# DaviGuanabara/dronechase

Measured on AMD Instinct MI355X. Metric: env-steps/sec (whole job), random-action rollout, higher is better.
Workload: dtype f32

## Files before the change

### dronechase_amd/csrc/te_engage_slots.hpp

```cpp
#pragma once
#include "te_engage.hpp"

namespace te {

constexpr int kSlotWaves = 16;
constexpr int kSlotPursuers = 4;

struct SlotRows {
  int D, P;
  TE_DEV int accS() const { return 0; }
  TE_DEV int accZone() const { return 1; }
  TE_DEV int accOrg() const { return 2; }
  TE_DEV int accOwn() const { return 3; }
  TE_DEV int pos(int k, int s) const { return 4 + k * D + s; }
  TE_DEV int cellr(int s) const { return 4 + 3 * D + 2 * s; }
  TE_DEV int npos(int k, int s) const { return 4 + (5 + k) * D + s; }
  TE_DEV int prec(int q) const { return 4 + 8 * D + q; }
  TE_DEV int prec2(int q) const { return 4 + 8 * D + 2 * q; }
};
__host__ __device__ inline int slot_lds_rows(int D, int P) { return 4 + 8 * D + 2 * P; }
enum : uint32_t { SLOT_HIT = 1u << 8, SLOT_EXPLODE = 1u << 9, SLOT_SUICIDE = 1u << 10 };

#define TE_SLOT_BARRIER() asm volatile("s_waitcnt lgkmcnt(0)\n\ts_barrier" ::: "memory")
#if defined(TE_DEBUG_STAMPS)
#define TE_WSTAMP(idx, wait)                                                                                              \
  do {                                                                                                                    \
    if (wait) asm volatile("s_waitcnt vmcnt(0) lgkmcnt(0)" ::: "memory");                                                 \
    if (p.dbg && s < 2 && lane == 0) p.dbg[64 + blockIdx.x * 16 + s * 8 + (idx)] = __builtin_amdgcn_s_memrealtime();     \
  } while (0)
#else
#define TE_WSTAMP(idx, wait) do {} while (0)
#endif

template <int DM>
__global__ __launch_bounds__(DM * 64) __attribute__((amdgpu_waves_per_eu(6, 10))) void engage_slots_kernel(Params p, const float* __restrict__ actions, StepOut o) {
  TE_EXACT
  extern __shared__ uint32_t sm[];
  const te_config& c = p.cfg;
  const int D = p.D, P = c.n_pursuers;
  const SlotRows R{D, P};
  const int lane = threadIdx.x & 63;
  const int s = __builtin_amdgcn_readfirstlane((int)(threadIdx.x >> 6));
  const int env = blockIdx.x * 64 + lane;
  const bool valid = env < p.N;
  const GView g{p.dstate, p.estate, D, p.Npad, env, P};
  const EnvIO io(p, env);
  const uint32_t pur_bits = (1u << P) - 1u, all_bits = (1u << D) - 1u, inv_bits = all_bits & ~pur_bits;
  const bool scripted = all_scripted(c);
  const bool is_p = s < P;
  auto L = [&](int row) -> uint32_t& { return sm[row * 64 + lane]; };
  auto Lf = [&](int row) { return __uint_as_float(sm[row * 64 + lane]); };
  auto Lor = [&](int row, uint32_t v) { __hip_atomic_fetch_or(&sm[row * 64 + lane], v, __ATOMIC_RELAXED, __HIP_MEMORY_SCOPE_WORKGROUP); };
  TE_WSTAMP(0, 0);

  const uint32_t* __restrict__ lm32 = reinterpret_cast<const uint32_t*>(p.live_mask);
  const uint32_t live = (uint32_t)__builtin_amdgcn_readfirstlane(lm32[2 * blockIdx.x]) & all_bits;
  const bool mine_live = is_p || ((live >> s) & 1u);
  auto next_round_of = [&](int r) { return r + (r < c.n_rounds ? 1 : c.n_rounds); };
  auto may_be_spawned = [&](int slot, int r) { const int i = slot - P; return i < invaders_in_round(c, next_round_of(r)) || i < invaders_in_round(c, 1); };
  if (!mine_live) {
    const int r = (int)io.le(TE_E_ROUND);
    if (__ballot(valid && may_be_spawned(s, r)) == 0ull) return;
  }
  float mx = io.ldf(TE_D_OBS_POS, s), my = io.ldf(TE_D_OBS_POS + 1, s), mz = io.ldf(TE_D_OBS_POS + 2, s);
  const uint32_t marmed_w = io.ld(TE_D_ARMED, s);
  const V3 apos{io.ldf(TE_D_OBS_POS, 0), io.ldf(TE_D_OBS_POS + 1, 0), io.ldf(TE_D_OBS_POS + 2, 0)};
  float ag[9];
#pragma unroll
  for (int k = 0; k < 3; ++k) ag[k] = io.ldf(TE_D_OBS_EULER + k, 0);
#pragma unroll
  for (int k = 3; k < 9; ++k) ag[k] = 0.0f;
  const uint32_t w_step = io.le(TE_E_STEP), w_max_step = io.le(TE_E_MAX_STEP), w_round = io.le(TE_E_ROUND), w_episode = io.le(TE_E_EPISODE);
  uint32_t w_last_dist = 0u, w_ak = 0u, w_lk = 0u, w_dd = 0u;
  float4 act = make_float4(0.0f, 0.0f, 0.0f, 0.0f);
  if (s == 0) {
#pragma unroll
    for (int k = 3; k < 9; ++k) ag[k] = io.ldf(TE_D_OBS_EULER + k, 0);
    w_last_dist = io.le(TE_E_LAST_DIST); w_ak = io.le(TE_E_AGENT_KILLS); w_lk = io.le(TE_E_ALLIES_KILLS); w_dd = io.le(TE_E_DEADS);
    if (valid) act = reinterpret_cast<const float4*>(actions)[env];
  }
  uint32_t w_mun = 0u, w_lf = 0u; float fx = 0.0f, fy = 0.0f, fz = 0.0f;
  if (is_p) {
    w_mun = io.ld(TE_D_MUNITION, s); w_lf = io.ld(TE_D_LAST_FIRED, s);
    fx = io.ldf(TE_D_FORMATION, s); fy = io.ldf(TE_D_FORMATION + 1, s); fz = io.ldf(TE_D_FORMATION + 2, s);
  }
  uint32_t zero = 0u;
  asm volatile("" : "+s"(zero));
  if (s == 0) { L(R.accS()) = 0u; L(R.accZone()) = 0u; L(R.accOrg()) = 0u; L(R.accOwn()) = 0u; }
  TE_SLOT_BARRIER();
  int step = (int)w_step + 1;
  int max_step = (int)w_max_step, round = (int)w_round;
  uint32_t episode = w_episode;
  int mun = (int)w_mun, lf = (int)w_lf;
  const float last_dist = __uint_as_float(w_last_dist);
  int agent_kills = (int)w_ak, allies_kills = (int)w_lk, deads = (int)w_dd;
  if (!mine_live) { mx = my = mz = 0.0f; }
  TE_WSTAMP(1, 1);

  const uint32_t a_me = (mine_live && marmed_w != zero && valid) ? 1u : 0u;
  {
    const float n = fnorm(V3{mx, my, mz});
    Lor(R.accS(), a_me << s); Lor(R.accZone(), (a_me & (n > c.dome_radius ? 1u : 0u)) << s); Lor(R.accOrg(), (a_me & (n < c.origin_range ? 1u : 0u)) << s);
    L(R.pos(0, s)) = __float_as_uint(mx); L(R.pos(1, s)) = __float_as_uint(my); L(R.pos(2, s)) = __float_as_uint(mz);
  }
  int cj = 0; float rh = 1.0f;
  if (s >= 1) {
    const M3 Rm = x_inverse_attitude(ag[0], ag[1], ag[2]);
    lidar_cell_fast(c, x_mul(Rm, sub(V3{mx, my, mz}, apos)), cj, rh);
    *reinterpret_cast<uint2*>(&sm[R.cellr(s) * 64 + 2 * lane]) = make_uint2((uint32_t)cj, __float_as_uint(rh));
  }
  TE_WSTAMP(2, 0);
  TE_SLOT_BARRIER();
  TE_WSTAMP(3, 0);
  const uint32_t S = L(R.accS()), zone = L(R.accZone()), org = L(R.accOrg());
  if (is_p) {
    int tgt = -1; float dmin = 0.0f;
    for (uint32_t m = live & inv_bits; m; m &= m - 1u) {
      const int j = __ffs((int)m) - 1;
      const float d = fdist(V3{mx, my, mz}, V3{Lf(R.pos(0, j)), Lf(R.pos(1, j)), Lf(R.pos(2, j))});
      const bool take = a_me != 0u && ((S >> j) & 1u) != 0u && (tgt < 0 || d < dmin);
      tgt = take ? j : tgt;
      dmin = take ? d : dmin;
    }
    uint32_t rec = (uint32_t)(tgt + 1);
    if (a_me && tgt >= 0 && dmin < c.shoot_range && gun_available(c, mun, lf, step) && mun > 0) {
      mun -= 1; lf = step;
      io.st(TE_D_MUNITION, s, (uint32_t)mun); io.st(TE_D_LAST_FIRED, s, (uint32_t)step);
      const U4 r = env_rng(c, env, RNG_HIT, (uint32_t)s, 0, episode, (uint32_t)step);
      if (u01(r.x) < c.hit_prob) {
        rec |= SLOT_HIT;
        if (c.evaluation) g.si(TE_D_KILLS, s, g.gi(TE_D_KILLS, s) + 1);
      }
    }
    if (a_me && tgt >= 0 && dmin < c.explosion_range) rec |= SLOT_EXPLODE | (mun == 0 ? SLOT_SUICIDE : 0u);
    L(R.prec(s)) = rec;
  }
  TE_SLOT_BARRIER();

  uint32_t killed = 0u;
  int agent_shots = 0, ally_shots = 0, exploded = 0, pursuer_suicided = 0, agent_suicided = 0;
  for (int q = 0; q < P; ++q) {
    const uint32_t r = L(R.prec(q));
    const int t = (int)(r & 0xFFu) - 1;
    if (r & SLOT_HIT) { killed |= 1u << t; if (q == 0) agent_shots += 1; else ally_shots += 1; }
    if (r & SLOT_EXPLODE) {
      killed |= (1u << q) | (1u << t);
      if ((r & SLOT_SUICIDE) && q == 0) agent_suicided += 1;
      else if (r & SLOT_SUICIDE) pursuer_suicided += 1;
      else exploded += 1;
    }
  }
  if ((!c.evaluation || (c.evaluation & TE_EVAL_ORIGIN_RULE)) && valid) killed |= org & inv_bits;
  const uint32_t A = S & ~killed;
  if ((killed >> s) & 1u) io.disarm(s);
  if (agent_shots + ally_shots > 0) max_step += c.step_increment;
  const int armed_invaders = __popc(A & inv_bits), armed_pursuers = __popc(A & pur_bits);
  const bool all_rounds_over = armed_invaders == 0 && round >= c.n_rounds;
  bool term;
  if (c.evaluation) term = (c.max_step > 0 && step > max_step) || all_rounds_over || zone != 0u || armed_pursuers == 0;
  else term = step > max_step || all_rounds_over || zone != 0u || armed_pursuers == 0 || (c.agent_death_terminates && !(A & 1u)) || apos.z < -5.99f;
  const bool to_terminal = valid && term && c.auto_reset;
  bool own = false;
  if (s >= 1) {
    own = ((A >> s) & 1u) != 0u && rh < 1.0f;
    for (uint32_t m = live & ~1u & ~(1u << s); m; m &= m - 1u) {
      const int k = __ffs((int)m) - 1;
      const uint2 cr = *reinterpret_cast<const uint2*>(&sm[R.cellr(k) * 64 + 2 * lane]);
      const float rk = __uint_as_float(cr.y);
      const bool beaten = ((A >> k) & 1u) != 0u && cr.x == (uint32_t)cj && (rk < rh || (rk == rh && k < s));
      own = own && !beaten;
    }
    if (own && valid) Lor(R.accOwn(), 1u << s);
  }
  const float flag_me = (float)(s < P ? TE_TYPE_LOYALWINGMAN : TE_TYPE_LOITERINGMUNITION) / 5.0f;
  const bool time_plane = c.lidar_channels != 2;
  auto patch = [&](float* dst) {
    dst += (size_t)env * lidar_words(c);
    dst[cj] = rh; dst[TE_LIDAR_CELLS + cj] = flag_me;
    if (time_plane) dst[2 * TE_LIDAR_CELLS + cj] = 0.1f;
  };
  if (valid && own && !to_terminal && o.obs.lidar) patch(o.obs.lidar);
  const unsigned long long term_b = __ballot(to_terminal);
  if (o.term.lidar && term_b && is_p) {
    for (unsigned long long tb = term_b; tb; tb &= tb - 1) {
      const int l = __ffsll((long long)tb) - 1;
      float* tile = o.term.lidar + (size_t)(blockIdx.x * 64 + l) * lidar_words(c);
      for (int e = s * 64 + lane; e < lidar_words(c); e += 64 * P) tile[e] = 1.0f;
    }
  }

  auto pos_of = [&](int t) { return V3{__uint_as_float(sm[R.pos(0, t) * 64 + lane]), __uint_as_float(sm[R.pos(1, t) * 64 + lane]), __uint_as_float(sm[R.pos(2, t) * 64 + lane])}; };
  if (s == 0) {
    if (valid) {
      io.stef(TE_E_LAST_ACTION + 0, act.x); io.stef(TE_E_LAST_ACTION + 1, act.y); io.stef(TE_E_LAST_ACTION + 2, act.z); io.stef(TE_E_LAST_ACTION + 3, act.w);
      io.ste(TE_E_STEP, (uint32_t)step);
      io.ste(TE_E_SNAP_MASK, S); io.ste(TE_E_SNAP_MASK_HI, 0u);
    }
    agent_kills += agent_shots; allies_kills += ally_shots; deads += exploded;
    if (to_terminal) {
      if (o.term.inertial) inertial_row_regs(c, o.term.inertial + (size_t)env * TE_OBS_INERTIAL_WORDS, mx, my, mz, ag, mun, lf, step);
      if (o.term.last_action) reinterpret_cast<float4*>(o.term.last_action)[env] = act;
    }
    float reward = 0.0f, cur_dist = last_dist;
    if (!c.evaluation) {
      float gs[3];
      gun_state(c, mun, lf, step, max_munition_of(c, 0), gs);
      const float dist_origin = fnorm(apos);
      int ally = -1;
      if ((S & 1u) && __popc(S & pur_bits) > 1) {
        float bd = 0.0f;
        for (int a = 1; a < P; ++a) {
          if ((S >> a) & 1u) {
            const float d = fdist(pos_of(a), apos);
            if (ally < 0 || d < bd) { ally = a; bd = d; }
          }
        }
      }
      const int chooser = ally < 0 ? 0 : ally;
      const int target = ((S >> chooser) & 1u) ? (int)(sm[R.prec(chooser) * 64 + lane] & 0xFFu) - 1 : -1;
      const V3 tp = target >= 0 ? pos_of(target) : V3{0.0f, 0.0f, 0.0f};
      cur_dist = fdist(apos, tp);
      const bool ready = gs[2] == 1.0f || gs[0] == 0.0f;
      float bonus = 0.0f, penalty = 0.0f;
      if (0.01f < last_dist - cur_dist && ready) bonus += c.approach_bonus_gain * fnorm(V3{ag[3], ag[4], ag[5]});
      const float score = ready ? -cur_dist : cur_dist * (2.0f * gs[1] - 1.0f);
      if (agent_shots > 0 || agent_suicided > 0) bonus += (float)(agent_shots + agent_suicided) * 1000.0f;
      if (ally_shots > 0 || pursuer_suicided > 0) bonus += 0.5f * (float)(ally_shots + pursuer_suicided) * 1000.0f;
      else if (exploded > 0) penalty += 1000.0f * (float)exploded;
      if (apos.z < -5.0f) penalty += (-5.0f - apos.z) * 1000.0f;
      if (zone & pur_bits) penalty += 1000.0f;
      if (dist_origin > c.born_radius - 2.0f) penalty += dist_origin - c.born_radius - 2.0f;
      reward = score + bonus - penalty;
    }
    if (valid) {
      if (!c.evaluation) io.stef(TE_E_LAST_DIST, cur_dist);
      io.ste(TE_E_AGENT_KILLS, (uint32_t)agent_kills); io.ste(TE_E_ALLIES_KILLS, (uint32_t)allies_kills); io.ste(TE_E_DEADS, (uint32_t)deads);
      if (agent_shots + ally_shots > 0) io.ste(TE_E_MAX_STEP, (uint32_t)max_step);
      o.reward[env] = reward;
      o.done[env] = term ? 1 : 0;
      reinterpret_cast<int4*>(o.info)[env] = make_int4(agent_kills, allies_kills, deads, round);
      io.ste(TE_E_INFO_WAVE, (uint32_t)round);
    }
  }

  uint32_t task = 0u;
  uint32_t snap_mask = S;
  auto mask_after_spawn = [&](int rnd, bool reset) {
    const uint32_t m = reset ? pur_bits : (A & pur_bits);
    const int n = invaders_in_round(c, rnd);
    return (uint32_t)(m | ((((1u << n) - 1u) << P) & all_bits));
  };
  if (valid && !term && armed_invaders == 0 && armed_pursuers > 0) {
    round = round + (round < c.n_rounds ? 1 : c.n_rounds);
    snap_mask = mask_after_spawn(round, false);
    if (s == 0) { io.ste(TE_E_ROUND, (uint32_t)round); io.ste(TE_E_SNAP_MASK, snap_mask); io.ste(TE_E_SNAP_MASK_HI, 0u); }
    task = (uint32_t)round;
  }
  if (to_terminal) {
    episode += 1u; step = 0; max_step = c.max_step; round = 1;
    snap_mask = mask_after_spawn(1, true);
    if (s == 0) {
      io.ste(TE_E_EPISODE, episode); io.ste(TE_E_STEP, 0u); io.ste(TE_E_MAX_STEP, (uint32_t)c.max_step); io.ste(TE_E_ROUND, 1u); io.ste(TE_E_INFO_WAVE, 1u);
      io.ste(TE_E_AGENT_KILLS, 0u); io.ste(TE_E_ALLIES_KILLS, 0u); io.ste(TE_E_DEADS, 0u);
      if (c.reward_model != TE_REWARD_L5_C1) io.stef(TE_E_LAST_DIST, c.dome_radius);
#pragma unroll
      for (int k = 0; k < 4; ++k) io.ste(TE_E_LAST_ACTION + k, 0u);
      io.ste(TE_E_SNAP_MASK, snap_mask); io.ste(TE_E_SNAP_MASK_HI, 0u);
    }
    act = make_float4(0.0f, 0.0f, 0.0f, 0.0f);
#pragma unroll
    for (int k = 0; k < 9; ++k) ag[k] = 0.0f;
    task = 1u | (1u << 8);
  }
  if (task != 0u) {
    const bool reset = (task >> 8) != 0u;
    V3 w{0.0f, 0.0f, 0.0f};
    const bool placed = io.spawn_uniform(c, env, s, (int)(task & 0xFFu), episode, reset, ((A >> s) & 1u) != 0u, w);
    if (placed) { mx = w.x; my = w.y; mz = w.z; }
    if (reset && is_p) { mun = max_munition_of(c, s); lf = -c.cooldown_steps; fx = mx; fy = my; fz = mz; }
  }
  if (s == 0 && __ballot(task != 0u) != 0ull) {
    for (uint32_t m = inv_bits & ~live; m; m &= m - 1u) {
      const int k2 = __ffs((int)m) - 1;
      if (__ballot(valid && may_be_spawned(k2, (int)w_round)) != 0ull) continue;
      if (task != 0u) io.st(TE_D_NAV_STATE, k2, (uint32_t)TE_NAV_WAIT);
    }
  }
  const uint32_t armed_post = task != 0u ? snap_mask : A;
  L(R.npos(0, s)) = __float_as_uint(mx); L(R.npos(1, s)) = __float_as_uint(my); L(R.npos(2, s)) = __float_as_uint(mz);
  if (o.term.lidar && term_b) asm volatile("s_waitcnt vmcnt(0)" ::: "memory");
  TE_WSTAMP(4, 0);
  TE_SLOT_BARRIER();
  TE_WSTAMP(5, 0);

  if (s >= 1 && to_terminal && own && o.term.lidar) patch(o.term.lidar);
  if (o.persist && o.obs.lidar && valid) {
    const uint32_t owners = L(R.accOwn());
    uint16_t* pv = o.prev + env;
    if (s == 0) pv[0] = (uint16_t)(to_terminal ? 0 : __popc(owners));
    else if (own && !to_terminal) pv[(size_t)(__popc(owners & ((1u << s) - 1u)) + 1) * p.Npad] = (uint16_t)cj;
  }
  if (s == 0) {
    if (o.obs.inertial && valid) inertial_row_regs(c, o.obs.inertial + (size_t)env * TE_OBS_INERTIAL_WORDS, mx, my, mz, ag, mun, lf, step);
    if (valid && o.obs.last_action) reinterpret_cast<float4*>(o.obs.last_action)[env] = act;
  }
  if (is_p && valid) {
    int first_skipped = -1;
    if (!scripted && !(armed_post & 1u)) first_skipped = (armed_post & pur_bits & ~1u) ? __ffs((int)(armed_post & pur_bits & ~1u)) - 1 : -1;
    io.stf(TE_X_REF + 0, s, mx); io.stf(TE_X_REF + 1, s, my); io.stf(TE_X_REF + 2, s, mz);
    if ((s > 0 || scripted) && ((armed_post >> s) & 1u) && s != first_skipped) {
      float out[3] = {0.0f, 0.0f, 0.0f};
      const bool ext = driven_externally(c, s);
      if (!ext && c.ally_policy == TE_ALLY_BT) {
        const V3 me{mx, my, mz};
        if (gun_available(c, mun, lf, step)) {
          int t = -1; float bd = 0.0f; V3 tp{0.0f, 0.0f, 0.0f};
          if ((snap_mask >> s) & 1u) {
            for (int j = P; j < D; ++j) {
              if (__ballot((snap_mask >> j) & 1u) == 0ull) continue;
              if ((snap_mask >> j) & 1u) {
                const V3 pj{Lf(R.npos(0, j)), Lf(R.npos(1, j)), Lf(R.npos(2, j))};
                const float d = fdist(me, pj);
                if (t < 0 || d < bd) { t = j; bd = d; tp = pj; }
              }
            }
          }
          x_cmd_toward(me, tp, c.ally_speed, out);
        } else x_cmd_toward(me, V3{fx, fy, fz}, c.ally_speed, out);
      } else if (ext || c.ally_policy != TE_ALLY_FROZEN) {
        out[0] = g.gf(TE_D_SETPOINT + 0, s); out[1] = g.gf(TE_D_SETPOINT + 1, s); out[2] = g.gf(TE_D_SETPOINT + 3, s);
      }
      io.stf(TE_X_CMD + 0, s, out[0]); io.stf(TE_X_CMD + 1, s, out[1]); io.stf(TE_X_CMD + 2, s, out[2]);
    }
  }
  const int writer = 0;
  if (s >= 1 || s == writer) {
    uint64_t dense = 0u, livem = 0u; int n = 0;
    uint16_t* items = p.mixed_items + (size_t)blockIdx.x * kMixedCap;
    const int k_last = s == writer ? D - 1 : s;
    for (int k = 0; k <= k_last; ++k) {
      const bool a = valid && ((armed_post >> k) & 1u) != 0u;
      const unsigned long long b = __ballot(a);
      const int cnt = __popcll(b);
      if (cnt == 0) continue;
      livem |= (uint64_t)1 << k;
      if (k == 0 || cnt >= p.dense_min || n + cnt > kMixedCap) { dense |= (uint64_t)1 << k; continue; }
      if (k == s && a) items[n + (int)__builtin_amdgcn_mbcnt_hi((uint32_t)(b >> 32), __builtin_amdgcn_mbcnt_lo((uint32_t)b, 0u))] = (uint16_t)(lane | (k << 8));
      n += cnt;
    }
    if (s == writer && lane == 0) { p.slot_mask[blockIdx.x] = dense; p.mixed_count[blockIdx.x] = (uint32_t)n; p.live_mask[blockIdx.x] = livem; }
  }
  TE_WSTAMP(6, 0);
  TE_WSTAMP(7, 1);
}

struct MultiSlotRows {
  int D, P, H;
  TE_DEV int accS(int h = 0) const { return h; }
  TE_DEV int accZone(int h = 0) const { return H + h; }
  TE_DEV int accOrg(int h = 0) const { return 2 * H + h; }
  TE_DEV int pos(int k, int s) const { return 3 * H + k * D + s; }
  TE_DEV int npos(int k, int s) const { return 3 * H + (3 + k) * D + s; }
  TE_DEV int prec(int q) const { return 3 * H + 6 * D + q; }
  TE_DEV int accOwn() const { return 3 * H + 6 * D + P; }
  TE_DEV int cellr(int s) const { return 3 * H + 1 + 6 * D + P + 2 * s; }
};
__host__ __device__ inline int multi_slot_lds_rows(int D, int P, bool lidar) { return 3 * (D > 32 ? 2 : 1) + 6 * D + P + (lidar ? 1 + 2 * D : 0); }

template <int SPW, bool LIDAR, bool WIDE = false>
__global__ __launch_bounds__(1024) __attribute__((amdgpu_waves_per_eu(SPW == 1 ? 4 : 6))) void engage_slots_multi_kernel(Params p, const float* __restrict__ actions, StepOut o) {
  TE_EXACT
  extern __shared__ uint32_t sm[];
  const te_config& c = p.cfg;
  const int D = p.D, P = c.n_pursuers;
  const int W = (int)(blockDim.x >> 6);
  using M = typename std::conditional<WIDE, uint64_t, uint32_t>::type;
  constexpr M one = 1;
  constexpr int kSh = WIDE ? 63 : 31;
  static_assert(!(WIDE && LIDAR), "the own sphere's owner row is 32 bits");
  const MultiSlotRows R{D, P, WIDE ? 2 : 1};
  auto popcM = [](M m) { return WIDE ? __popcll((unsigned long long)m) : __popc((uint32_t)m); };
  auto ffsM = [](M m) { return WIDE ? __ffsll((long long)m) - 1 : __ffs((int)(uint32_t)m) - 1; };
  const int lane = threadIdx.x & 63;
  const int s = __builtin_amdgcn_readfirstlane((int)(threadIdx.x >> 6));
  const int env = blockIdx.x * 64 + lane;
  const bool valid = env < p.N;
  const GView g{p.dstate, p.estate, D, p.Npad, env, P};
  const EnvIO io(p, env);
  const M pur_bits = (one << P) - one, all_bits = D >= (int)(8 * sizeof(M)) ? ~(M)0 : (one << D) - one, inv_bits = all_bits & ~pur_bits;
  const bool scripted = all_scripted(c);
  const bool is_p = s < P;
  int sl[SPW]; bool has[SPW];
#pragma unroll
  for (int u = 0; u < SPW; ++u) { sl[u] = s + u * W; has[u] = sl[u] < D; }
  auto L = [&](int row) -> uint32_t& { return sm[row * 64 + lane]; };
  auto Lf = [&](int row) { return __uint_as_float(sm[row * 64 + lane]); };
  auto Lor = [&](int row, uint32_t v) { __hip_atomic_fetch_or(&sm[row * 64 + lane], v, __ATOMIC_RELAXED, __HIP_MEMORY_SCOPE_WORKGROUP); };
  TE_WSTAMP(0, 0);

  const uint32_t* __restrict__ lm32 = reinterpret_cast<const uint32_t*>(p.live_mask);
  const M live = (WIDE ? (M)((uint64_t)(uint32_t)__builtin_amdgcn_readfirstlane(lm32[2 * blockIdx.x]) | ((uint64_t)(uint32_t)__builtin_amdgcn_readfirstlane(lm32[2 * blockIdx.x + 1]) << 32))
                       : (M)(uint32_t)__builtin_amdgcn_readfirstlane(lm32[2 * blockIdx.x])) & all_bits;
  auto next_round_of = [&](int r) { return r + (r < c.n_rounds ? 1 : c.n_rounds); };
// ... 639 lines not shown
```

### dronechase_amd/csrc/te_env.hip

```cpp
#include <hip/hip_runtime.h>
#include <hip/hip_ext.h>

#include <algorithm>
#include <cmath>
#include <cstdio>
#include <cstdlib>
#include <cstring>
#include <new>
#include <string>
#include <tuple>
#include <type_traits>
#include <vector>

#include "te_logic.hpp"
#include "te_stacked.hpp"
#include "te_stackview.hpp"
#include "te_engage.hpp"
#include "te_engage_slots.hpp"
#include "te_policy.hpp"
#include "te_wingman.hpp"
#include "te_policy_grad.hpp"
#include "te_policy_opt.hpp"
#include "te_rollout.hpp"
#include "te_monitor.hpp"
// ... 666 lines not shown
  if (cfg->task == TE_TASK_STAGE01 && !(cfg->n_pursuers == 2 && cfg->n_invaders == 1)) return "te_create: stage01 is 2 pursuers + 1 invader";
  if (cfg->lidar_radius <= 0.0f || cfg->dome_radius <= 0.0f || cfg->max_speed <= 0.0f) return "te_create: radii / max_speed must be positive";
  if (cfg->control_every_substep != 0 && cfg->control_every_substep != 1) return "te_create: control_every_substep is 0 or 1";
  if (cfg->lidar_channels != 3 && cfg->lidar_channels != 2) return "te_create: lidar_channels is 3 (distance, flag, time) or 2 (distance, flag)";
  if (cfg->lidar_channels == 2 && cfg->stacked_obs) return "te_create: the stacked observation (level5) always has 3 channels";
  if (cfg->io_location != TE_IO_DEVICE && cfg->io_location != TE_IO_HOST) return "te_create: io_location is TE_IO_DEVICE or TE_IO_HOST";
  if (cfg->io_location == TE_IO_HOST && (cfg->stacked_obs || cfg->ally_policy == TE_ALLY_EXTERNAL || ((uint32_t)cfg->evaluation >> 8) != 0u))
    return "te_create: TE_IO_HOST serves te_reset / te_observe / te_step / te_random_actions / te_get_state / te_set_state; the stacked observation and caller-driven wingmen take device pointers";
  if (cfg->drone_contact != 0 && cfg->drone_contact != 1) return "te_create: drone_contact is 0 or 1";
  if (cfg->drone_contact && !(cfg->contact_radius > 0.0f)) return "te_create: contact_radius must be positive";
  const size_t npad = ((size_t)cfg->n_envs + 63) / 64 * 64;
  if ((size_t)(TE_DRONE_WORDS + TE_X_WORDS) * D * npad >= (1ull << 30)) return "te_create: n_envs * drones too large for one te_env (state planes are indexed with 32 bits); shard it";
  return nullptr;
}

static const char* plan_kernels(const te_config& c, KernelPlan* out, size_t multi_lds_max = 160 * 1024) {
  KernelPlan& k = *out = KernelPlan{};
  const int P = c.n_pursuers, D = P + c.n_invaders, fam = family_of(c.task);
  const long long chunks = (c.n_envs + 63) / 64;
  const bool l4 = fam == FAM_LEVEL4, contact = c.drone_contact != 0;
  const char* engage = getenv("TE_ENGAGE");
  const bool eng_lds = engage && !strcmp(engage, "lds"), eng_regs = engage && !strcmp(engage, "regs");
  const bool regs_l4 = l4 && !eng_lds && P <= 7 && D <= 37;
  const bool regs_s2 = fam == FAM_STAGE02 && !eng_lds && P <= 2 && D <= 10;
  const bool regs_s1 = fam == FAM_STAGE01 && !eng_lds;
  if (D > kMaxD && !(regs_l4 && c.stacked_obs))
    return "te_create: more than 32 drones per env are served for the stacked-observation tasks only (te_step_stacked / te_step_students: stacked_obs, P <= 7, P + I <= 37)";
  if ((c.agent_scripted || c.reward_model != TE_REWARD_EXP03 || !c.agent_death_terminates || c.initial_invaders != 1 || c.invaders_per_round != 1) && !regs_l4)
    return "te_create: agent_scripted / reward_model / agent_death_terminates / the round rule are built into engage_kernel: the level4 task family with P <= 7 and P + I <= 37";
  if (contact && !(regs_l4 && P <= 6 && D <= 18))
    return "te_create: cfg.drone_contact is built into engage_kernel: the level4 task family with P <= 6 and P + I <= 18";
#ifdef TE_DEBUG_STAMPS
  if (contact) return "te_create: cfg.drone_contact is not served by the stamp build (TE_DEBUG_STAMPS leaves out the drone-contact engage kernels)";
#endif
  const bool slots = regs_l4 && !eng_regs && !c.stacked_obs && D <= kSlotWaves && P <= kSlotPursuers && c.reward_model == TE_REWARD_EXP03 && !contact;
  int spw = 0;
  const size_t multi_lds = (size_t)multi_slot_lds_rows(D, P, !c.stacked_obs) * 256;
  if (regs_l4 && !eng_regs && (D <= 32 || (c.stacked_obs && D <= 3 * kSlotWaves)) && !contact && (c.stacked_obs || D > kSlotWaves || slots)) {
    int s = D <= kSlotWaves ? 1 : D <= 2 * kSlotWaves ? 2 : 3;
    const int spw_max = c.stacked_obs ? 3 : 2;
    while (c.stacked_obs && s < spw_max && chunks * ((D + s - 1) / s) > 256 * 24 && P <= (D + s) / (s + 1)) s += 1;
    if (const char* v = getenv("TE_SLOT_SPW")) { const int n = atoi(v); if (n >= 1 && n <= spw_max && (D + n - 1) / n <= kSlotWaves) s = n; }
    if (P <= (D + s - 1) / s && multi_lds <= multi_lds_max && (c.stacked_obs || s > 1)) spw = s;
  }
  const size_t lds = (size_t)lds_rows(D, P) * kEPB * sizeof(uint32_t), slot_lds = (size_t)slot_lds_rows(D, P) * 256;
  const unsigned multi_block = spw ? 64u * (unsigned)((D + spw - 1) / spw) : 0u;
  static_assert(kSlotWaves == 16 && kPushSplit == 4 && FAM_LEVEL4 == 0 && FAM_STAGE01 == 1 && FAM_STAGE02 == 2, "the kernel names below");
  if (spw && D > 32) k.engage = {TE_KERNEL(engage_slots_multi_kernel<3, false, true>), multi_block, multi_lds};
  else if (spw && !c.stacked_obs) k.engage = {TE_KERNEL(engage_slots_multi_kernel<2, true, false>), multi_block, multi_lds};
  else if (spw == 1) k.engage = {TE_KERNEL(engage_slots_multi_kernel<1, false, false>), multi_block, multi_lds};
  else if (spw == 2) k.engage = {TE_KERNEL(engage_slots_multi_kernel<2, false, false>), multi_block, multi_lds};
  else if (spw == 3) k.engage = {TE_KERNEL(engage_slots_multi_kernel<3, false, false>), multi_block, multi_lds};
  else if (regs_s2 && !eng_regs) k.engage = {TE_KERNEL(engage_slots_stage02_kernel<16>), 64u * D, slot_lds};
  else if (slots) k.engage = {TE_KERNEL(engage_slots_kernel<16>), 64u * D, slot_lds};
#ifndef TE_DEBUG_STAMPS
  else if (contact && P <= 2 && D <= 11) k.engage = {TE_KERNEL(engage_kernel<2, 9, true>), 64, 0};
  else if (contact) k.engage = {TE_KERNEL(engage_kernel<6, 12, true>), 64, 0};
#endif
  else if (regs_l4 && P <= 2 && D <= 11) k.engage = {TE_KERNEL(engage_kernel<2, 9, false>), 64, 0};
  else if (regs_l4 && P <= 6 && D <= 18) k.engage = {TE_KERNEL(engage_kernel<6, 12, false>), 64, 0};
  else if (regs_l4) k.engage = {TE_KERNEL(engage_kernel<7, 30, false>), 64, 0};
  else if (regs_s2) k.engage = {TE_KERNEL(engage_stage02_kernel<2, 8>), 64, 0};
  else if (regs_s1) k.engage = {TE_KERNEL(engage_stage01_kernel), 64, 0};
  else if (l4 && lds > 53 * 1024) k.engage = {TE_KERNEL(engage_observe_kernel<0, 512>), 512, lds};
  else if (l4) k.engage = {TE_KERNEL(engage_observe_kernel<0, 256>), 256, lds};
  else if (fam == FAM_STAGE01) k.engage = {TE_KERNEL(engage_observe_kernel<1, 256>), 256, lds};
  else k.engage = {TE_KERNEL(engage_observe_kernel<2, 256>), 256, lds};
  k.observe_lds = lds;
  k.records_cells = !c.stacked_obs && (regs_l4 || regs_s2 || regs_s1);
  const bool help_ok = c.motor_noise && c.substeps >= 2 && c.substeps <= 48 && P <= kEagerP;
  const bool typical_light = l4 && chunks * std::min(D, P + 2) <= 1280;
  bool help = help_ok && ((long long)c.n_envs * D <= kHelpMaxPairs || typical_light);
  if (const char* v = getenv("TE_K1_HELP")) help = atoi(v) != 0 && help_ok;
  launch_by_family(fam, [&](auto F) { with_bool(c.motor_noise != 0, [&](auto N) { with_bool(c.control_every_substep != 0, [&](auto C) { with_bool(help, [&](auto H) {
    constexpr int kF = decltype(F)::value;
    constexpr bool kN = decltype(N)::value, kC = decltype(C)::value, kH = decltype(H)::value;
    if constexpr (kN || !kH) k.substeps[0] = substep_role<kF, kN, false, kC, kH>(c), k.substeps[1] = substep_role<kF, kN, true, kC, kH>(c);
  }); }); }); });
  if (const char* v = getenv("TE_DENSE_MIN")) { const int n = atoi(v); if (n >= 1 && n <= 65) k.dense_min = n; }
  if (c.stacked_obs) k.n_fill_waves = 512;
  if (const char* v = getenv("TE_FILL_WAVES")) { const int n = atoi(v); if (n >= 1 && n <= (1 << 20)) k.n_fill_waves = n; }
  if (c.stacked_obs) {
    const char* stacked = getenv("TE_STACKED");
    const int dm = stacked && !strcmp(stacked, "lds") ? 0 : D <= 18 ? 18 : D <= 37 ? 37 : 0;
    bool split = dm == 18 && chunks * P * kPushSplit <= 4096;
    if (const char* v = getenv("TE_PUSH_SPLIT")) split = dm == 18 && atoi(v) != 0;
    const size_t view_lds = (size_t)view_lds_rows(D) * kEPB * sizeof(uint32_t);
    if (dm == 18 && split) k.ring_push = {TE_KERNEL(ring_push_kernel<18, 4>), 64 * kPushSplit, (size_t)4 * 18 * 256};
    else if (dm == 18) k.ring_push = {TE_KERNEL(ring_push_kernel<18, 1>), 64, 0};
    else if (dm == 37) k.ring_push = {TE_KERNEL(ring_push_kernel<37, 1>), 64, 0};
    if (dm == 18) k.stack_view = {TE_KERNEL(stack_view_kernel<18>), kViewThreads, view_lds};
    else if (dm == 37) k.stack_view = {TE_KERNEL(stack_view_kernel<37>), kViewThreads, view_lds};
    else k.stack_view = {TE_KERNEL(stacked_kernel), kStackThreads, (size_t)stack_lds_rows(D, P) * kEPB * sizeof(uint32_t)};
    k.records_cells = dm != 0;
  }
  if (c.ally_policy == TE_ALLY_EXTERNAL || ((uint32_t)c.evaluation >> 8) != 0u) {
    const size_t n_floats = (size_t)c.n_envs * lidar_words(c);
    k.wingman_one = {TE_KERNEL(observe_ally_kernel), 256, 0};
    if (c.n_envs >= 4096 && (n_floats & 3) == 0 && (n_floats >> 2) < (1ull << 32)) {
      k.wingman_view = {TE_KERNEL(ally_view_kernel), 64, 0};
      k.wingman_patch = {TE_KERNEL(ally_patch_kernel), 256, 0};
    }
  }
  return nullptr;
}

struct te_env {
// ... 918 lines not shown
```

Baseline: 902.2 million.

## Pack invader slots onto a fixed number of waves in engage_slots_kernel

The slot engage kernel used to launch one wave per drone slot. It now launches P pursuer waves plus a fixed number of invader waves (default 4), and each invader wave handles several invader slots round-robin. Per-slot work (loads, lidar cell, ownership, spawn, persistence, item emission) becomes loops over the wave's slot mask. This shrinks the block and cuts barrier and launch cost for large D, at the price of serialising invader work within a wave and adding register arrays per slot.

```diff
diff --git a/dronechase_amd/csrc/te_engage_slots.hpp b/dronechase_amd/csrc/te_engage_slots.hpp
--- a/dronechase_amd/csrc/te_engage_slots.hpp
+++ b/dronechase_amd/csrc/te_engage_slots.hpp
@@ -26,11 +26,19 @@
 #define TE_WSTAMP(idx, wait)                                                                                              \
   do {                                                                                                                    \
     if (wait) asm volatile("s_waitcnt vmcnt(0) lgkmcnt(0)" ::: "memory");                                                 \
-    if (p.dbg && s < 2 && lane == 0) p.dbg[64 + blockIdx.x * 16 + s * 8 + (idx)] = __builtin_amdgcn_s_memrealtime();     \
+    const int wv_ = (int)(threadIdx.x >> 6);                                                                              \
+    if (p.dbg && wv_ < 2 && lane == 0) p.dbg[64 + blockIdx.x * 16 + wv_ * 8 + (idx)] = __builtin_amdgcn_s_memrealtime(); \
   } while (0)
 #else
 #define TE_WSTAMP(idx, wait) do {} while (0)
 #endif
+
+#ifndef TE_SLOT_INVADER_WAVES
+#define TE_SLOT_INVADER_WAVES 4
+#endif
+constexpr int kSlotInvaderWaves = TE_SLOT_INVADER_WAVES;
+constexpr int kSlotsPerInvaderWave = (kSlotWaves - 1 + kSlotInvaderWaves - 1) / kSlotInvaderWaves;
+__host__ __device__ inline int slot_waves(int D, int P) { return D < P + kSlotInvaderWaves ? D : P + kSlotInvaderWaves; }
 
 template <int DM>
 __global__ __launch_bounds__(DM * 64) __attribute__((amdgpu_waves_per_eu(6, 10))) void engage_slots_kernel(Params p, const float* __restrict__ actions, StepOut o) {
@@ -40,14 +48,15 @@
   const int D = p.D, P = c.n_pursuers;
   const SlotRows R{D, P};
   const int lane = threadIdx.x & 63;
-  const int s = __builtin_amdgcn_readfirstlane((int)(threadIdx.x >> 6));
+  const int w = __builtin_amdgcn_readfirstlane((int)(threadIdx.x >> 6));
+  const int n_inv_waves = (int)(blockDim.x >> 6) - P;
   const int env = blockIdx.x * 64 + lane;
   const bool valid = env < p.N;
   const GView g{p.dstate, p.estate, D, p.Npad, env, P};
   const EnvIO io(p, env);
   const uint32_t pur_bits = (1u << P) - 1u, all_bits = (1u << D) - 1u, inv_bits = all_bits & ~pur_bits;
   const bool scripted = all_scripted(c);
-  const bool is_p = s < P;
+  const bool is_p = w < P;
   auto L = [&](int row) -> uint32_t& { return sm[row * 64 + lane]; };
   auto Lf = [&](int row) { return __uint_as_float(sm[row * 64 + lane]); };
   auto Lor = [&](int row, uint32_t v) { __hip_atomic_fetch_or(&sm[row * 64 + lane], v, __ATOMIC_RELAXED, __HIP_MEMORY_SCOPE_WORKGROUP); };
@@ -55,25 +64,49 @@
 
   const uint32_t* __restrict__ lm32 = reinterpret_cast<const uint32_t*>(p.live_mask);
   const uint32_t live = (uint32_t)__builtin_amdgcn_readfirstlane(lm32[2 * blockIdx.x]) & all_bits;
-  const bool mine_live = is_p || ((live >> s) & 1u);
+  const uint32_t w_round = io.le(TE_E_ROUND), w_step = io.le(TE_E_STEP), w_max_step = io.le(TE_E_MAX_STEP), w_episode = io.le(TE_E_EPISODE);
+  const V3 apos{io.ldf(TE_D_OBS_POS, 0), io.ldf(TE_D_OBS_POS + 1, 0), io.ldf(TE_D_OBS_POS + 2, 0)};
+  float ag[9];
+#pragma unroll
+  for (int k = 0; k < 3; ++k) ag[k] = io.ldf(TE_D_OBS_EULER + k, 0);
+#pragma unroll
+  for (int k = 3; k < 9; ++k) ag[k] = 0.0f;
   auto next_round_of = [&](int r) { return r + (r < c.n_rounds ? 1 : c.n_rounds); };
   auto may_be_spawned = [&](int slot, int r) { const int i = slot - P; return i < invaders_in_round(c, next_round_of(r)) || i < invaders_in_round(c, 1); };
-  if (!mine_live) {
-    const int r = (int)io.le(TE_E_ROUND);
-    if (__ballot(valid && may_be_spawned(s, r)) == 0ull) return;
-  }
-  float mx = io.ldf(TE_D_OBS_POS, s), my = io.ldf(TE_D_OBS_POS + 1, s), mz = io.ldf(TE_D_OBS_POS + 2, s);
-  const uint32_t marmed_w = io.ld(TE_D_ARMED, s);
-  const V3 apos{io.ldf(TE_D_OBS_POS, 0), io.ldf(TE_D_OBS_POS + 1, 0), io.ldf(TE_D_OBS_POS + 2, 0)};
-  float ag[9];
-#pragma unroll
-  for (int k = 0; k < 3; ++k) ag[k] = io.ldf(TE_D_OBS_EULER + k, 0);
-#pragma unroll
-  for (int k = 3; k < 9; ++k) ag[k] = 0.0f;
-  const uint32_t w_step = io.le(TE_E_STEP), w_max_step = io.le(TE_E_MAX_STEP), w_round = io.le(TE_E_ROUND), w_episode = io.le(TE_E_EPISODE);
+  uint32_t mine = 1u << w;
+  if (!is_p) {
+    uint32_t cand = live & inv_bits;
+    for (uint32_t m = inv_bits & ~live; m; m &= m - 1u) {
+      const int k = __ffs((int)m) - 1;
+      if (__ballot(valid && may_be_spawned(k, (int)w_round)) != 0ull) cand |= 1u << k;
+    }
+    mine = 0u;
+    int turn = 0;
+    for (uint32_t m = cand; m; m &= m - 1u) {
+      if (turn == w - P) mine |= m & (0u - m);
+      turn = turn + 1 == n_inv_waves ? 0 : turn + 1;
+    }
+    if (mine == 0u) return;
+  }
+  int sl[kSlotsPerInvaderWave];
+  float mx[kSlotsPerInvaderWave], my[kSlotsPerInvaderWave], mz[kSlotsPerInvaderWave];
+  uint32_t marmed_w[kSlotsPerInvaderWave];
+  {
+    uint32_t m = mine;
+#pragma unroll
+    for (int u = 0; u < kSlotsPerInvaderWave; ++u) {
+      sl[u] = m ? __ffs((int)m) - 1 : -1;
+      m &= m - 1u;
+      mx[u] = my[u] = mz[u] = 0.0f; marmed_w[u] = 0u;
+      if (u == 0 || sl[u] >= 0) {
+        mx[u] = io.ldf(TE_D_OBS_POS, sl[u]); my[u] = io.ldf(TE_D_OBS_POS + 1, sl[u]); mz[u] = io.ldf(TE_D_OBS_POS + 2, sl[u]);
+        marmed_w[u] = io.ld(TE_D_ARMED, sl[u]);
+      }
+    }
+  }
   uint32_t w_last_dist = 0u, w_ak = 0u, w_lk = 0u, w_dd = 0u;
   float4 act = make_float4(0.0f, 0.0f, 0.0f, 0.0f);
-  if (s == 0) {
+  if (w == 0) {
 #pragma unroll
     for (int k = 3; k < 9; ++k) ag[k] = io.ldf(TE_D_OBS_EULER + k, 0);
     w_last_dist = io.le(TE_E_LAST_DIST); w_ak = io.le(TE_E_AGENT_KILLS); w_lk = io.le(TE_E_ALLIES_KILLS); w_dd = io.le(TE_E_DEADS);
@@ -81,12 +114,12 @@
   }
   uint32_t w_mun = 0u, w_lf = 0u; float fx = 0.0f, fy = 0.0f, fz = 0.0f;
   if (is_p) {
-    w_mun = io.ld(TE_D_MUNITION, s); w_lf = io.ld(TE_D_LAST_FIRED, s);
-    fx = io.ldf(TE_D_FORMATION, s); fy = io.ldf(TE_D_FORMATION + 1, s); fz = io.ldf(TE_D_FORMATION + 2, s);
+    w_mun = io.ld(TE_D_MUNITION, w); w_lf = io.ld(TE_D_LAST_FIRED, w);
+    fx = io.ldf(TE_D_FORMATION, w); fy = io.ldf(TE_D_FORMATION + 1, w); fz = io.ldf(TE_D_FORMATION + 2, w);
   }
   uint32_t zero = 0u;
   asm volatile("" : "+s"(zero));
-  if (s == 0) { L(R.accS()) = 0u; L(R.accZone()) = 0u; L(R.accOrg()) = 0u; L(R.accOwn()) = 0u; }
+  if (w == 0) { L(R.accS()) = 0u; L(R.accZone()) = 0u; L(R.accOrg()) = 0u; L(R.accOwn()) = 0u; }
   TE_SLOT_BARRIER();
   int step = (int)w_step + 1;
   int max_step = (int)w_max_step, round = (int)w_round;
@@ -94,30 +127,49 @@
   int mun = (int)w_mun, lf = (int)w_lf;
   const float last_dist = __uint_as_float(w_last_dist);
   int agent_kills = (int)w_ak, allies_kills = (int)w_lk, deads = (int)w_dd;
-  if (!mine_live) { mx = my = mz = 0.0f; }
   TE_WSTAMP(1, 1);
 
-  const uint32_t a_me = (mine_live && marmed_w != zero && valid) ? 1u : 0u;
+  auto pos_of = [&](int t) { return V3{__uint_as_float(sm[R.pos(0, t) * 64 + lane]), __uint_as_float(sm[R.pos(1, t) * 64 + lane]), __uint_as_float(sm[R.pos(2, t) * 64 + lane])}; };
   {
-    const float n = fnorm(V3{mx, my, mz});
-    Lor(R.accS(), a_me << s); Lor(R.accZone(), (a_me & (n > c.dome_radius ? 1u : 0u)) << s); Lor(R.accOrg(), (a_me & (n < c.origin_range ? 1u : 0u)) << s);
-    L(R.pos(0, s)) = __float_as_uint(mx); L(R.pos(1, s)) = __float_as_uint(my); L(R.pos(2, s)) = __float_as_uint(mz);
-  }
-  int cj = 0; float rh = 1.0f;
-  if (s >= 1) {
-    const M3 Rm = x_inverse_attitude(ag[0], ag[1], ag[2]);
-    lidar_cell_fast(c, x_mul(Rm, sub(V3{mx, my, mz}, apos)), cj, rh);
-    *reinterpret_cast<uint2*>(&sm[R.cellr(s) * 64 + 2 * lane]) = make_uint2((uint32_t)cj, __float_as_uint(rh));
+    uint32_t a_bits = 0u;
+#pragma unroll
+    for (int u = 0; u < kSlotsPerInvaderWave; ++u) {
+      if (sl[u] >= 0) {
+        const int s = sl[u];
+        const bool slot_live = is_p || ((live >> s) & 1u) != 0u;
+        if (!slot_live) { mx[u] = my[u] = mz[u] = 0.0f; }
+        a_bits |= ((slot_live && marmed_w[u] != zero && valid) ? 1u : 0u) << s;
+        L(R.pos(0, s)) = __float_as_uint(mx[u]); L(R.pos(1, s)) = __float_as_uint(my[u]); L(R.pos(2, s)) = __float_as_uint(mz[u]);
+      }
+    }
+    uint32_t zone_bits = 0u, org_bits = 0u;
+    M3 Rm{};
+    if (w >= 1) Rm = x_inverse_attitude(ag[0], ag[1], ag[2]);
+    for (uint32_t m = mine; m; m &= m - 1u) {
+      const int s = __ffs((int)m) - 1;
+      const V3 me = pos_of(s);
+      const float n = fnorm(me);
+      const uint32_t a_me = (a_bits >> s) & 1u;
+      zone_bits |= (a_me & (n > c.dome_radius ? 1u : 0u)) << s; org_bits |= (a_me & (n < c.origin_range ? 1u : 0u)) << s;
+      if (s >= 1) {
+        int cj = 0; float rh = 1.0f;
+        lidar_cell_fast(c, x_mul(Rm, sub(me, apos)), cj, rh);
+        *reinterpret_cast<uint2*>(&sm[R.cellr(s) * 64 + 2 * lane]) = make_uint2((uint32_t)cj, __float_as_uint(rh));
+      }
+    }
+    Lor(R.accS(), a_bits); Lor(R.accZone(), zone_bits); Lor(R.accOrg(), org_bits);
   }
   TE_WSTAMP(2, 0);
   TE_SLOT_BARRIER();
   TE_WSTAMP(3, 0);
   const uint32_t S = L(R.accS()), zone = L(R.accZone()), org = L(R.accOrg());
   if (is_p) {
+    const V3 me = pos_of(w);
+    const uint32_t a_me = (S >> w) & 1u;
     int tgt = -1; float dmin = 0.0f;
     for (uint32_t m = live & inv_bits; m; m &= m - 1u) {
       const int j = __ffs((int)m) - 1;
-      const float d = fdist(V3{mx, my, mz}, V3{Lf(R.pos(0, j)), Lf(R.pos(1, j)), Lf(R.pos(2, j))});
+      const float d = fdist(me, pos_of(j));
       const bool take = a_me != 0u && ((S >> j) & 1u) != 0u && (tgt < 0 || d < dmin);
       tgt = take ? j : tgt;
       dmin = take ? d : dmin;
@@ -125,15 +177,15 @@
     uint32_t rec = (uint32_t)(tgt + 1);
     if (a_me && tgt >= 0 && dmin < c.shoot_range && gun_available(c, mun, lf, step) && mun > 0) {
       mun -= 1; lf = step;
-      io.st(TE_D_MUNITION, s, (uint32_t)mun); io.st(TE_D_LAST_FIRED, s, (uint32_t)step);
-      const U4 r = env_rng(c, env, RNG_HIT, (uint32_t)s, 0, episode, (uint32_t)step);
+      io.st(TE_D_MUNITION, w, (uint32_t)mun); io.st(TE_D_LAST_FIRED, w, (uint32_t)step);
+      const U4 r = env_rng(c, env, RNG_HIT, (uint32_t)w, 0, episode, (uint32_t)step);
       if (u01(r.x) < c.hit_prob) {
         rec |= SLOT_HIT;
-        if (c.evaluation) g.si(TE_D_KILLS, s, g.gi(TE_D_KILLS, s) + 1);
+        if (c.evaluation) g.si(TE_D_KILLS, w, g.gi(TE_D_KILLS, w) + 1);
       }
     }
     if (a_me && tgt >= 0 && dmin < c.explosion_range) rec |= SLOT_EXPLODE | (mun == 0 ? SLOT_SUICIDE : 0u);
-    L(R.prec(s)) = rec;
+    L(R.prec(w)) = rec;
   }
   TE_SLOT_BARRIER();
 
@@ -152,7 +204,6 @@
   }
   if ((!c.evaluation || (c.evaluation & TE_EVAL_ORIGIN_RULE)) && valid) killed |= org & inv_bits;
   const uint32_t A = S & ~killed;
-  if ((killed >> s) & 1u) io.disarm(s);
   if (agent_shots + ally_shots > 0) max_step += c.step_increment;
   const int armed_invaders = __popc(A & inv_bits), armed_pursuers = __popc(A & pur_bits);
   const bool all_rounds_over = armed_invaders == 0 && round >= c.n_rounds;
@@ -160,37 +211,40 @@
   if (c.evaluation) term = (c.max_step > 0 && step > max_step) || all_rounds_over || zone != 0u || armed_pursuers == 0;
   else term = step > max_step || all_rounds_over || zone != 0u || armed_pursuers == 0 || (c.agent_death_terminates && !(A & 1u)) || apos.z < -5.99f;
   const bool to_terminal = valid && term && c.auto_reset;
-  bool own = false;
-  if (s >= 1) {
-    own = ((A >> s) & 1u) != 0u && rh < 1.0f;
-    for (uint32_t m = live & ~1u & ~(1u << s); m; m &= m - 1u) {
-      const int k = __ffs((int)m) - 1;
-      const uint2 cr = *reinterpret_cast<const uint2*>(&sm[R.cellr(k) * 64 + 2 * lane]);
-      const float rk = __uint_as_float(cr.y);
-      const bool beaten = ((A >> k) & 1u) != 0u && cr.x == (uint32_t)cj && (rk < rh || (rk == rh && k < s));
-      own = own && !beaten;
-    }
-    if (own && valid) Lor(R.accOwn(), 1u << s);
-  }
-  const float flag_me = (float)(s < P ? TE_TYPE_LOYALWINGMAN : TE_TYPE_LOITERINGMUNITION) / 5.0f;
   const bool time_plane = c.lidar_channels != 2;
-  auto patch = [&](float* dst) {
+  auto patch = [&](float* dst, int cj, float rh, int s) {
     dst += (size_t)env * lidar_words(c);
-    dst[cj] = rh; dst[TE_LIDAR_CELLS + cj] = flag_me;
+    dst[cj] = rh; dst[TE_LIDAR_CELLS + cj] = (float)(s < P ? TE_TYPE_LOYALWINGMAN : TE_TYPE_LOITERINGMUNITION) / 5.0f;
     if (time_plane) dst[2 * TE_LIDAR_CELLS + cj] = 0.1f;
   };
-  if (valid && own && !to_terminal && o.obs.lidar) patch(o.obs.lidar);
+  for (uint32_t m2 = mine; m2; m2 &= m2 - 1u) {
+    const int s = __ffs((int)m2) - 1;
+    if ((killed >> s) & 1u) io.disarm(s);
+    if (s >= 1) {
+      const uint2 mc = *reinterpret_cast<const uint2*>(&sm[R.cellr(s) * 64 + 2 * lane]);
+      const int cj = (int)mc.x; const float rh = __uint_as_float(mc.y);
+      bool own = ((A >> s) & 1u) != 0u && rh < 1.0f;
+      for (uint32_t m = live & ~1u & ~(1u << s); m; m &= m - 1u) {
+        const int k = __ffs((int)m) - 1;
+        const uint2 cr = *reinterpret_cast<const uint2*>(&sm[R.cellr(k) * 64 + 2 * lane]);
+        const float rk = __uint_as_float(cr.y);
+        const bool beaten = ((A >> k) & 1u) != 0u && cr.x == (uint32_t)cj && (rk < rh || (rk == rh && k < s));
+        own = own && !beaten;
+      }
+      if (own && valid) Lor(R.accOwn(), 1u << s);
+      if (valid && own && !to_terminal && o.obs.lidar) patch(o.obs.lidar, cj, rh, s);
+    }
+  }
   const unsigned long long term_b = __ballot(to_terminal);
   if (o.term.lidar && term_b && is_p) {
     for (unsigned long long tb = term_b; tb; tb &= tb - 1) {
       const int l = __ffsll((long long)tb) - 1;
       float* tile = o.term.lidar + (size_t)(blockIdx.x * 64 + l) * lidar_words(c);
-      for (int e = s * 64 + lane; e < lidar_words(c); e += 64 * P) tile[e] = 1.0f;
-    }
-  }
-
-  auto pos_of = [&](int t) { return V3{__uint_as_float(sm[R.pos(0, t) * 64 + lane]), __uint_as_float(sm[R.pos(1, t) * 64 + lane]), __uint_as_float(sm[R.pos(2, t) * 64 + lane])}; };
-  if (s == 0) {
+      for (int e = w * 64 + lane; e < lidar_words(c); e += 64 * P) tile[e] = 1.0f;
+    }
+  }
+
+  if (w == 0) {
     if (valid) {
       io.stef(TE_E_LAST_ACTION + 0, act.x); io.stef(TE_E_LAST_ACTION + 1, act.y); io.stef(TE_E_LAST_ACTION + 2, act.z); io.stef(TE_E_LAST_ACTION + 3, act.w);
       io.ste(TE_E_STEP, (uint32_t)step);
@@ -198,7 +252,8 @@
     }
     agent_kills += agent_shots; allies_kills += ally_shots; deads += exploded;
     if (to_terminal) {
-      if (o.term.inertial) inertial_row_regs(c, o.term.inertial + (size_t)env * TE_OBS_INERTIAL_WORDS, mx, my, mz, ag, mun, lf, step);
+      const V3 me = pos_of(0);
+      if (o.term.inertial) inertial_row_regs(c, o.term.inertial + (size_t)env * TE_OBS_INERTIAL_WORDS, me.x, me.y, me.z, ag, mun, lf, step);
       if (o.term.last_action) reinterpret_cast<float4*>(o.term.last_action)[env] = act;
     }
     float reward = 0.0f, cur_dist = last_dist;
@@ -253,13 +308,13 @@
   if (valid && !term && armed_invaders == 0 && armed_pursuers > 0) {
     round = round + (round < c.n_rounds ? 1 : c.n_rounds);
     snap_mask = mask_after_spawn(round, false);
-    if (s == 0) { io.ste(TE_E_ROUND, (uint32_t)round); io.ste(TE_E_SNAP_MASK, snap_mask); io.ste(TE_E_SNAP_MASK_HI, 0u); }
+    if (w == 0) { io.ste(TE_E_ROUND, (uint32_t)round); io.ste(TE_E_SNAP_MASK, snap_mask); io.ste(TE_E_SNAP_MASK_HI, 0u); }
     task = (uint32_t)round;
   }
   if (to_terminal) {
     episode += 1u; step = 0; max_step = c.max_step; round = 1;
     snap_mask = mask_after_spawn(1, true);
-    if (s == 0) {
+    if (w == 0) {
       io.ste(TE_E_EPISODE, episode); io.ste(TE_E_STEP, 0u); io.ste(TE_E_MAX_STEP, (uint32_t)c.max_step); io.ste(TE_E_ROUND, 1u); io.ste(TE_E_INFO_WAVE, 1u);
       io.ste(TE_E_AGENT_KILLS, 0u); io.ste(TE_E_ALLIES_KILLS, 0u); io.ste(TE_E_DEADS, 0u);
       if (c.reward_model != TE_REWARD_L5_C1) io.stef(TE_E_LAST_DIST, c.dome_radius);
@@ -272,14 +327,19 @@
     for (int k = 0; k < 9; ++k) ag[k] = 0.0f;
     task = 1u | (1u << 8);
   }
-  if (task != 0u) {
-    const bool reset = (task >> 8) != 0u;
-    V3 w{0.0f, 0.0f, 0.0f};
-    const bool placed = io.spawn_uniform(c, env, s, (int)(task & 0xFFu), episode, reset, ((A >> s) & 1u) != 0u, w);
-    if (placed) { mx = w.x; my = w.y; mz = w.z; }
-    if (reset && is_p) { mun = max_munition_of(c, s); lf = -c.cooldown_steps; fx = mx; fy = my; fz = mz; }
-  }
-  if (s == 0 && __ballot(task != 0u) != 0ull) {
+  for (uint32_t m2 = mine; m2; m2 &= m2 - 1u) {
+    const int s = __ffs((int)m2) - 1;
+    V3 me = pos_of(s);
+    if (task != 0u) {
+      const bool reset = (task >> 8) != 0u;
+      V3 at{0.0f, 0.0f, 0.0f};
+      const bool placed = io.spawn_uniform(c, env, s, (int)(task & 0xFFu), episode, reset, ((A >> s) & 1u) != 0u, at);
+      if (placed) me = at;
+      if (reset && is_p) { mun = max_munition_of(c, s); lf = -c.cooldown_steps; fx = me.x; fy = me.y; fz = me.z; }
+    }
+    L(R.npos(0, s)) = __float_as_uint(me.x); L(R.npos(1, s)) = __float_as_uint(me.y); L(R.npos(2, s)) = __float_as_uint(me.z);
+  }
+  if (w == 0 && __ballot(task != 0u) != 0ull) {
     for (uint32_t m = inv_bits & ~live; m; m &= m - 1u) {
       const int k2 = __ffs((int)m) - 1;
       if (__ballot(valid && may_be_spawned(k2, (int)w_round)) != 0ull) continue;
@@ -287,35 +347,42 @@
     }
   }
   const uint32_t armed_post = task != 0u ? snap_mask : A;
-  L(R.npos(0, s)) = __float_as_uint(mx); L(R.npos(1, s)) = __float_as_uint(my); L(R.npos(2, s)) = __float_as_uint(mz);
   if (o.term.lidar && term_b) asm volatile("s_waitcnt vmcnt(0)" ::: "memory");
   TE_WSTAMP(4, 0);
   TE_SLOT_BARRIER();
   TE_WSTAMP(5, 0);
 
-  if (s >= 1 && to_terminal && own && o.term.lidar) patch(o.term.lidar);
-  if (o.persist && o.obs.lidar && valid) {
+  {
     const uint32_t owners = L(R.accOwn());
-    uint16_t* pv = o.prev + env;
-    if (s == 0) pv[0] = (uint16_t)(to_terminal ? 0 : __popc(owners));
-    else if (own && !to_terminal) pv[(size_t)(__popc(owners & ((1u << s) - 1u)) + 1) * p.Npad] = (uint16_t)cj;
-  }
-  if (s == 0) {
-    if (o.obs.inertial && valid) inertial_row_regs(c, o.obs.inertial + (size_t)env * TE_OBS_INERTIAL_WORDS, mx, my, mz, ag, mun, lf, step);
+    const bool persist = o.persist && o.obs.lidar && valid;
+    if ((o.term.lidar && term_b) || persist) {
+      for (uint32_t m2 = mine; m2; m2 &= m2 - 1u) {
+        const int s = __ffs((int)m2) - 1;
+        const bool own = ((owners >> s) & 1u) != 0u;
+        uint16_t* pv = o.prev + env;
+        if (s == 0) { if (persist) pv[0] = (uint16_t)(to_terminal ? 0 : __popc(owners)); continue; }
+        const uint2 mc = *reinterpret_cast<const uint2*>(&sm[R.cellr(s) * 64 + 2 * lane]);
+        if (to_terminal && own && o.term.lidar) patch(o.term.lidar, (int)mc.x, __uint_as_float(mc.y), s);
+        if (persist && own && !to_terminal) pv[(size_t)(__popc(owners & ((1u << s) - 1u)) + 1) * p.Npad] = (uint16_t)mc.x;
+      }
+    }
+  }
+  const V3 me{Lf(R.npos(0, w < P ? w : 0)), Lf(R.npos(1, w < P ? w : 0)), Lf(R.npos(2, w < P ? w : 0))};
+  if (w == 0) {
+    if (o.obs.inertial && valid) inertial_row_regs(c, o.obs.inertial + (size_t)env * TE_OBS_INERTIAL_WORDS, me.x, me.y, me.z, ag, mun, lf, step);
     if (valid && o.obs.last_action) reinterpret_cast<float4*>(o.obs.last_action)[env] = act;
   }
   if (is_p && valid) {
     int first_skipped = -1;
     if (!scripted && !(armed_post & 1u)) first_skipped = (armed_post & pur_bits & ~1u) ? __ffs((int)(armed_post & pur_bits & ~1u)) - 1 : -1;
-    io.stf(TE_X_REF + 0, s, mx); io.stf(TE_X_REF + 1, s, my); io.stf(TE_X_REF + 2, s, mz);
-    if ((s > 0 || scripted) && ((armed_post >> s) & 1u) && s != first_skipped) {
+    io.stf(TE_X_REF + 0, w, me.x); io.stf(TE_X_REF + 1, w, me.y); io.stf(TE_X_REF + 2, w, me.z);
+    if ((w > 0 || scripted) && ((armed_post >> w) & 1u) && w != first_skipped) {
       float out[3] = {0.0f, 0.0f, 0.0f};
-      const bool ext = driven_externally(c, s);
+      const bool ext = driven_externally(c, w);
       if (!ext && c.ally_policy == TE_ALLY_BT) {
-        const V3 me{mx, my, mz};
         if (gun_available(c, mun, lf, step)) {
           int t = -1; float bd = 0.0f; V3 tp{0.0f, 0.0f, 0.0f};
-          if ((snap_mask >> s) & 1u) {
+          if ((snap_mask >> w) & 1u) {
             for (int j = P; j < D; ++j) {
               if (__ballot((snap_mask >> j) & 1u) == 0ull) continue;
               if ((snap_mask >> j) & 1u) {
@@ -328,16 +395,15 @@
           x_cmd_toward(me, tp, c.ally_speed, out);
         } else x_cmd_toward(me, V3{fx, fy, fz}, c.ally_speed, out);
       } else if (ext || c.ally_policy != TE_ALLY_FROZEN) {
-        out[0] = g.gf(TE_D_SETPOINT + 0, s); out[1] = g.gf(TE_D_SETPOINT + 1, s); out[2] = g.gf(TE_D_SETPOINT + 3, s);
-      }
-      io.stf(TE_X_CMD + 0, s, out[0]); io.stf(TE_X_CMD + 1, s, out[1]); io.stf(TE_X_CMD + 2, s, out[2]);
-    }
-  }
-  const int writer = 0;
-  if (s >= 1 || s == writer) {
+        out[0] = g.gf(TE_D_SETPOINT + 0, w); out[1] = g.gf(TE_D_SETPOINT + 1, w); out[2] = g.gf(TE_D_SETPOINT + 3, w);
+      }
+      io.stf(TE_X_CMD + 0, w, out[0]); io.stf(TE_X_CMD + 1, w, out[1]); io.stf(TE_X_CMD + 2, w, out[2]);
+    }
+  }
+  {
     uint64_t dense = 0u, livem = 0u; int n = 0;
     uint16_t* items = p.mixed_items + (size_t)blockIdx.x * kMixedCap;
-    const int k_last = s == writer ? D - 1 : s;
+    const int k_last = w == 0 ? D - 1 : 31 - __clz((int)mine);
     for (int k = 0; k <= k_last; ++k) {
       const bool a = valid && ((armed_post >> k) & 1u) != 0u;
       const unsigned long long b = __ballot(a);
@@ -345,10 +411,10 @@
       if (cnt == 0) continue;
       livem |= (uint64_t)1 << k;
       if (k == 0 || cnt >= p.dense_min || n + cnt > kMixedCap) { dense |= (uint64_t)1 << k; continue; }
-      if (k == s && a) items[n + (int)__builtin_amdgcn_mbcnt_hi((uint32_t)(b >> 32), __builtin_amdgcn_mbcnt_lo((uint32_t)b, 0u))] = (uint16_t)(lane | (k << 8));
+      if (((mine >> k) & 1u) && a) items[n + (int)__builtin_amdgcn_mbcnt_hi((uint32_t)(b >> 32), __builtin_amdgcn_mbcnt_lo((uint32_t)b, 0u))] = (uint16_t)(lane | (k << 8));
       n += cnt;
     }
-    if (s == writer && lane == 0) { p.slot_mask[blockIdx.x] = dense; p.mixed_count[blockIdx.x] = (uint32_t)n; p.live_mask[blockIdx.x] = livem; }
+    if (w == 0 && lane == 0) { p.slot_mask[blockIdx.x] = dense; p.mixed_count[blockIdx.x] = (uint32_t)n; p.live_mask[blockIdx.x] = livem; }
   }
   TE_WSTAMP(6, 0);
   TE_WSTAMP(7, 1);
diff --git a/dronechase_amd/csrc/te_env.hip b/dronechase_amd/csrc/te_env.hip
--- a/dronechase_amd/csrc/te_env.hip
+++ b/dronechase_amd/csrc/te_env.hip
@@ -742,7 +742,7 @@
   else if (spw == 2) k.engage = {TE_KERNEL(engage_slots_multi_kernel<2, false, false>), multi_block, multi_lds};
   else if (spw == 3) k.engage = {TE_KERNEL(engage_slots_multi_kernel<3, false, false>), multi_block, multi_lds};
   else if (regs_s2 && !eng_regs) k.engage = {TE_KERNEL(engage_slots_stage02_kernel<16>), 64u * D, slot_lds};
-  else if (slots) k.engage = {TE_KERNEL(engage_slots_kernel<16>), 64u * D, slot_lds};
+  else if (slots) k.engage = {TE_KERNEL(engage_slots_kernel<16>), 64u * (unsigned)slot_waves(D, P), slot_lds};
 #ifndef TE_DEBUG_STAMPS
   else if (contact && P <= 2 && D <= 11) k.engage = {TE_KERNEL(engage_kernel<2, 9, true>), 64, 0};
   else if (contact) k.engage = {TE_KERNEL(engage_kernel<6, 12, true>), 64, 0};
```

New measurement: 883.2 million. 2.1% lower.
